# nz0001na/MorphGANformer

Measured on AMD Instinct MI355X. Metric: latent-projection iters/sec @1024^2, k=17 latents, higher is better.
Workload: dtype f32; 1 GPU; configs[1]: single 1024x1024 face per GPU, Wing+LPIPS(squeeze)+MSE literal-mode projection step, noise_mode=random, seeded synthetic weights/targets/landmarks; k=17, z_dim=32, targets_per_gpu=1, parallelism=pair-sharded x1, graph_replay=True, loss_generator_overlap=True, steps_per_forward=32

## Files before the change

### include/mgf.h

```cpp
#ifndef MGF_H_
#define MGF_H_

#include <stdint.h>

#ifdef __cplusplus
extern "C" {
#endif

typedef void* mgf_stream_t;

enum { MGF_OK = 0, MGF_EINVAL = -1, MGF_EUNSUPPORTED = -2, MGF_ELAUNCH = -3, MGF_ETOOBIG = -4 };
enum { MGF_F32 = 0, MGF_F64 = 1, MGF_F16 = 2 };
enum { MGF_FILTER_SEPARABLE = 2 };
enum { MGF_FILTER_LARGE = 4 };
enum { MGF_ACT_LINEAR = 1, MGF_ACT_RELU = 2, MGF_ACT_LRELU = 3, MGF_ACT_TANH = 4, MGF_ACT_SIGMOID = 5,
       MGF_ACT_ELU = 6, MGF_ACT_SELU = 7, MGF_ACT_SOFTPLUS = 8, MGF_ACT_SWISH = 9,
       MGF_ACT_RELU_POST = 10 };

const char* mgf_last_error(void);
int mgf_version(void);
int mgf_device_ok(void);

int mgf_bias_act(void* y, const void* x, const void* b, const void* xref, const void* yref, const void* dy,
                 int dtype, int64_t numel, int64_t step_b, int64_t size_b,
// ... 80 lines not shown

int mgf_conv3x3s2_few_inputs_f32(float* y, const float* x, const float* w, const float* bias, int32_t n, int32_t cin, int32_t in_h,
                                 int32_t in_w, int32_t cout, int32_t relu, mgf_stream_t stream);
int mgf_tconv3x3s2_few_outputs_f32(float* y, const float* x, const float* wp, int32_t n, int32_t cin, int32_t h, int32_t w, int32_t cout,
                                   int32_t cout_pad, int32_t pitch, int64_t y_plane, int64_t y_batch, mgf_stream_t stream);
int mgf_conv3x3_winograd3_up2res_f32(float* y, const float* x, const float* u, const float* in_scale, const float* out_scale,
                                     const float* residual_low, int32_t n, int32_t cin, int32_t h, int32_t w, int32_t cout,
                                     int32_t out_scale_stride, const mgf_epilogue* ep, mgf_stream_t stream);
int mgf_winograd3_force_shape(int32_t shape);
int mgf_conv3x3_winograd3_rgb_f32(float* rgb_out, const float* x, const float* u, const float* in_scale, const float* out_scale,
                                  const float* rgb_w, const float* rgb_bias, int32_t n, int32_t cin, int32_t h, int32_t w, int32_t cout,
                                  int32_t out_scale_stride, int32_t rgb_channels, mgf_stream_t stream);
int mgf_conv3x3_winograd_f32(float* y, const float* x, const float* u, const float* in_scale, const float* out_scale, int32_t n,
                             int32_t cin, int32_t h, int32_t w, int32_t cout, int32_t out_scale_stride, const mgf_epilogue* ep,
                             mgf_stream_t stream);

int mgf_tconv3x3s2_border_f32(float* t, const float* x, const float* wp, const float* in_scale, const float* out_scale, int32_t n,
                              int32_t cin, int32_t h, int32_t w, int32_t cout, int32_t cout_pad, int64_t t_pitch, int64_t t_plane,
                              int64_t t_batch, int64_t out_scale_stride, mgf_stream_t stream);

int mgf_tconv3x3s2_winograd_f32(float* t, const float* x, const float* u, const float* in_scale, const float* out_scale, int32_t n,
                                int32_t cin, int32_t h, int32_t w, int32_t cout, int32_t pitch, int64_t t_plane, int64_t t_batch,
                                int64_t out_scale_stride, mgf_stream_t stream);
int mgf_tconv_winograd_weights_f32(float* u, const float* w, int32_t cout, int32_t cin, double gain, mgf_stream_t stream);

int mgf_pack_conv_weights(float* wp, float* wsq, const float* w, int32_t cout, int32_t cin, int32_t kh, int32_t kw,
                          int32_t cout_pad, float gain, int32_t flip, mgf_stream_t stream);

typedef struct mgf_style_job {
    const float* aff_w;
    const float* aff_b;
    const float* wsq;
    float* s;
    float* d;
    int32_t cin, cout;
    int32_t w_offset;
    float aff_gain, style_gain;
} mgf_style_job;
int mgf_demod_f32(float* d, const float* s, const float* wsq, int32_t n, int32_t cin, int32_t cout, mgf_stream_t stream);
int mgf_demod_bwd_f32(float* ds, const float* dd, const float* d, const float* s, const float* wsq, int32_t n, int32_t cin, int32_t cout,
                      mgf_stream_t stream);
int mgf_style_demod(const mgf_style_job* job, const float* ws, int64_t ws_stride_n, int32_t n, int32_t wdim, mgf_stream_t stream);
int mgf_style_demod_multi(const mgf_style_job* jobs_dev, int32_t njobs, const float* ws, int64_t ws_stride_n,
                          int32_t n, int32_t wdim, int32_t max_cin, mgf_stream_t stream);

int mgf_duplex_attention(float* y, const float* x, const float* wqc, const float* spos, const float* vwb,
// ... 199 lines not shown
```

### morphganformer_amd/_lib.py

```python
from __future__ import annotations

import ctypes as C
import os

import torch

HERE = os.path.dirname(os.path.abspath(__file__))
LIB_PATH = os.environ.get("MGF_LIB_PATH") or os.path.join(HERE, "libmgf_hip.so")

MGF_F32, MGF_F64, MGF_F16 = 0, 1, 2
ACT_IDS = {"linear": 1, "relu": 2, "lrelu": 3, "tanh": 4, "sigmoid": 5, "elu": 6, "selu": 7, "softplus": 8, "swish": 9,
           "relu_post": 10}
MAX_TAPS = 9

i32, i64, f32, f64, vp = C.c_int32, C.c_int64, C.c_float, C.c_double, C.c_void_p


class Epilogue(C.Structure):
    _fields_ = [("bias", vp), ("noise", vp), ("noise_strength", vp), ("noise_n", i32), ("act", i32), ("alpha", f32),
                ("gain", f32), ("residual", vp)]


class ConvDesc(C.Structure):
    _fields_ = [("n", i32), ("cin", i32), ("in_h", i32), ("in_w", i32), ("cout", i32), ("cout_pad", i32),
# ... 36 lines not shown
    "mgf_version": (C.c_int, []),
    "mgf_device_ok": (C.c_int, []),
    "mgf_bias_act": (C.c_int, [vp, vp, vp, vp, vp, vp, C.c_int, i64, i64, i64, C.c_int, C.c_int, f32, f32, f32, vp]),
    "mgf_upfirdn2d": (C.c_int, [vp, vp, vp, C.c_int, i32, i32, i32, i32, i64, i64, i64, i64, i32, i32, i64, i64, i64, i64,
                                i32, i32, i32, i32, i32, i32, i32, i32, i32, i32, i32, f32, C.POINTER(Epilogue), vp]),
    "mgf_conv_taps_f32": (C.c_int, [vp, vp, vp, vp, vp, C.POINTER(ConvDesc), C.POINTER(Epilogue), vp]),
    "mgf_conv_taps_bf16x3_f32": (C.c_int, [vp, vp, vp, vp, vp, C.POINTER(ConvDesc), C.POINTER(Epilogue), vp]),
    "mgf_tconv3x3s2_border_f32": (C.c_int, [vp, vp, vp, vp, vp, i32, i32, i32, i32, i32, i32, i64, i64, i64, i64, vp]),
    "mgf_tconv3x3s2_winograd_f32": (C.c_int, [vp, vp, vp, vp, vp, i32, i32, i32, i32, i32, i32, i64, i64, i64, vp]),
    "mgf_tconv_winograd_weights_f32": (C.c_int, [vp, vp, i32, i32, C.c_double, vp]),
    "mgf_winograd_weights_f32": (C.c_int, [vp, vp, i32, i32, f32, vp]),
    "mgf_conv3x3_winograd_f32": (C.c_int, [vp, vp, vp, vp, vp, i32, i32, i32, i32, i32, i32, C.POINTER(Epilogue), vp]),
    "mgf_winograd2_weights_f32": (C.c_int, [vp, vp, i32, i32, f32, vp]),
    "mgf_conv3x3_winograd2_f32": (C.c_int, [vp, vp, vp, vp, vp, i32, i32, i32, i32, i32, i32, C.POINTER(Epilogue), vp]),
    "mgf_conv3x3_winograd2_rgb_f32": (C.c_int, [vp, vp, vp, vp, vp, vp, vp, i32, i32, i32, i32, i32, i32, i32, vp]),
    "mgf_conv3x3_winograd3_f32": (C.c_int, [vp, vp, vp, vp, vp, i32, i32, i32, i32, i32, i32, C.POINTER(Epilogue), vp]),
    "mgf_conv1x1_f32": (C.c_int, [vp, vp, vp, vp, i32, i32, i32, i32, i32, i64, i32, C.POINTER(Epilogue), vp]),
    "mgf_conv3x3s2_few_inputs_f32": (C.c_int, [vp, vp, vp, vp, i32, i32, i32, i32, i32, i32, vp]),
    "mgf_tconv3x3s2_few_outputs_f32": (C.c_int, [vp, vp, vp, i32, i32, i32, i32, i32, i32, i32, i64, i64, vp]),
    "mgf_conv1x1_force_shape": (C.c_int, [i32]),
    "mgf_conv3x3_winograd3_slice_f32": (C.c_int, [vp, vp, vp, vp, vp, i32, i32, i32, i32, i32, i32, i64, i32, C.POINTER(Epilogue), vp]),
    "mgf_conv3x3_winograd3_up2res_f32": (C.c_int, [vp, vp, vp, vp, vp, vp, i32, i32, i32, i32, i32, i32, C.POINTER(Epilogue), vp]),
    "mgf_winograd3_force_shape": (C.c_int, [i32]),
    "mgf_conv3x3_winograd3_rgb_f32": (C.c_int, [vp, vp, vp, vp, vp, vp, vp, i32, i32, i32, i32, i32, i32, i32, vp]),
    "mgf_conv3x3_winograd2_slice_f32": (C.c_int, [vp, vp, vp, vp, vp, i32, i32, i32, i32, i32, i32, i64, i32, C.POINTER(Epilogue), vp]),
    "mgf_pack_conv_weights": (C.c_int, [vp, vp, vp, i32, i32, i32, i32, i32, f32, i32, vp]),
    "mgf_conv_profile_begin": (C.c_int, []),
    "mgf_conv_profile_end": (C.c_int, [C.POINTER(ConvProfRec), i32]),
    "mgf_demod_f32": (C.c_int, [vp, vp, vp, i32, i32, i32, vp]),
    "mgf_demod_bwd_f32": (C.c_int, [vp, vp, vp, vp, vp, i32, i32, i32, vp]),
    "mgf_style_demod": (C.c_int, [C.POINTER(StyleJob), vp, i64, i32, i32, vp]),
    "mgf_style_demod_multi": (C.c_int, [vp, i32, vp, i64, i32, i32, i32, vp]),
    "mgf_duplex_attention": (C.c_int, [vp, vp, vp, vp, vp, i32, i32, i32, i32, C.POINTER(Epilogue), i32, vp, vp, vp]),
    "mgf_att_map_upsample_f32": (C.c_int, [vp, vp, i32, i32, i32, i32, i32, i32, vp]),
    "mgf_attn_values": (C.c_int, [C.POINTER(AttnJob), vp, i64, i64, i32, i32, i32, vp]),
    "mgf_attn_values_multi": (C.c_int, [vp, i32, vp, i64, i64, i32, i32, i32, vp]),
    "mgf_randn_f32": (C.c_int, [vp, i64, C.c_uint64, vp, vp]),
    "mgf_rgb_weights_f32": (C.c_int, [vp, vp, vp, i32, i32, i32, vp]),
    "mgf_torgb_compose_weights_f32": (C.c_int, [vp, vp, vp, vp, vp, vp, i32, i32, i32, i32, vp]),
    "mgf_conv3x3_few_outputs_f32": (C.c_int, [vp, vp, vp, vp, i32, i32, i32, i32, i32, vp]),
    "mgf_mapping_param_floats": (i64, [i32, i32, i32]),
    "mgf_mapping_forward": (C.c_int, [vp, vp, vp, i32, i32, i32, i32, i32, vp]),
    "mgf_reduce_scratch_floats": (i64, []),
    "mgf_mse_f32": (C.c_int, [vp, vp, vp, i32, i64, i64, f32, i32, vp, vp]),
    "mgf_dssim_scratch_bytes": (i64, [i32, i32, i32, i32]),
    "mgf_dssim_u8_f32": (C.c_int, [vp, vp, vp, i32, i32, i32, i32, i64, f32, f32, i32, vp, vp]),
# ... 131 lines not shown
```

### morphganformer_amd/conv.py

```python
from __future__ import annotations

import ctypes as C
import os
from dataclasses import dataclass

import torch

from . import _lib


def round_up(v: int, m: int) -> int:
    return (v + m - 1) // m * m


def profile_begin():
    _lib.check(_lib.lib().mgf_conv_profile_begin(), "conv_profile_begin")


def profile_end(max_recs=4096):
    recs = (_lib.ConvProfRec * max_recs)()
    n = _lib.lib().mgf_conv_profile_end(recs, max_recs)
    if n < 0:
        _lib.check(n, "conv_profile_end")
    return [(recs[i].kernel.decode(), recs[i].flops, recs[i].seconds, recs[i].ksplit, recs[i].bytes) for i in range(min(n, max_recs))]
# ... 370 lines not shown
                                                      _lib.stream_ptr()), "conv3x3_few_outputs")
    return out


TCONV_WINO = os.environ.get("MGF_TCONV_WINO", "1") != "0"
TCONV_WINO_MIN_WGS = 4096


def tconv_winograd_weights(w: torch.Tensor, gain: float = 1.0) -> torch.Tensor:
    _lib.require_gpu(w)
    w = w.contiguous().float()
    cout, cin, kh, kw = w.shape
    assert (kh, kw) == (3, 3) and cin % 4 == 0
    u = torch.empty([25, cin // 4, cout, 4], dtype=torch.float32, device=w.device)
    _lib.check(_lib.lib().mgf_tconv_winograd_weights_f32(u.data_ptr(), w.data_ptr(), cout, cin, float(gain), _lib.stream_ptr()),
               "tconv_winograd_weights")
    return u


def tconv_winograd_ok(n, cin, h, w, cout, out, bf=None) -> bool:
    return bool(TCONV_WINO and SPLIT_TCONV_BORDER and bf is None and h % 2 == 0 and w % 2 == 0 and min(h, w) >= TCONV_SPLIT_MIN and cin % 4 == 0 and cout % 32 == 0
                and out.shape[3] % 4 == 0 and out.data_ptr() % 16 == 0
                and n * -(-h // 4) * -(-w // 32) * (cout // 32) >= TCONV_WINO_MIN_WGS)


def tconv3x3s2_forward(x, pc: PackedConv, in_scale=None, out_scale=None, out=None, bf=None, wt=None):
    _lib.require_gpu(x, pc.wp, in_scale, out_scale, out, wt)
    assert pc.kh == 3 and pc.kw == 3 and x.dtype == torch.float32 and x.is_contiguous()
    n, cin, h, w = x.shape
    oh, ow = 2 * h + 1, 2 * w + 1
    if out is None:
        out = torch.empty([n, pc.cout, oh, tconv_pitch(w)], dtype=torch.float32, device=x.device)
    pitch = out.shape[3]
    assert out.is_contiguous() and tuple(out.shape) == (n, pc.cout, oh, pitch) and pitch >= ow and pitch % 4 == 0
    if NARROW_CONV and pc.cout <= 4 and in_scale is None and out_scale is None:
        rc = _lib.lib().mgf_tconv3x3s2_few_outputs_f32(out.data_ptr(), x.data_ptr(), pc.wp.data_ptr(), n, cin, h, w, pc.cout, pc.cout_pad,
                                                       pitch, oh * pitch, pc.cout * oh * pitch, _lib.stream_ptr())
        _lib.check(rc, "tconv3x3s2_few_outputs")
        return out[:, :, :, :ow]
    if wt is not None and tconv_winograd_ok(n, cin, h, w, pc.cout, out, bf):
        assert tuple(wt.shape) == (25, cin // 4, pc.cout, 4)
        os_stride = 0 if out_scale is None else out_scale.stride(0) if out_scale.ndim == 2 else 0
        rc = _lib.lib().mgf_tconv3x3s2_winograd_f32(out.data_ptr(), x.data_ptr(), wt.data_ptr(), _lib.ptr(in_scale), _lib.ptr(out_scale), n, cin, h,
                                                    w, pc.cout, pitch, oh * pitch, pc.cout * oh * pitch, os_stride, _lib.stream_ptr())
        _lib.check(rc, "tconv3x3s2_winograd")
        rc = _lib.lib().mgf_tconv3x3s2_border_f32(out.data_ptr(), x.data_ptr(), pc.wp.data_ptr(), _lib.ptr(in_scale), _lib.ptr(out_scale),
# ... 41 lines not shown
```

### morphganformer_amd/csrc/wino_tconv.hip

```cpp
#include "mgf_common.h"
#include <algorithm>
#include <type_traits>

namespace {

typedef float f32x16 __attribute__((ext_vector_type(16)));
typedef float v2f __attribute__((ext_vector_type(2)));

constexpr int WTCK = 4;
constexpr int WTFW = 34;
constexpr int WTFH = 5;
constexpr int WTFP = WTFH * WTFW;
constexpr int WTNP = 25;
constexpr int WTXS = 14;
__constant__ float wt_ones[WTCK] = {1.f, 1.f, 1.f, 1.f};

struct WinoTParams {
    float* t;
    const float* x;
    const float* u;
    const float* in_scale;
    const float* out_scale;
    int n, cin, h, w, cout, os_stride, pitch;
    int tiles_x, tiles_y, co_tiles;
    int xcd_per;
    int64_t t_plane, t_batch;
};

__global__ __launch_bounds__(256, 2) void wino_tconv_kernel(WinoTParams p) {
    constexpr int CST = 256, RAW = WTCK * CST;
    extern __shared__ float lds[];
    float* const raw0 = lds;
    float* const raw1 = raw0 + RAW;
    const int tid = threadIdx.x, lane = tid & 63;
    const int a = __builtin_amdgcn_readfirstlane(tid >> 6);
    const int l31 = lane & 31, half = lane >> 5;
    const int tx = l31 & 15, ty = l31 >> 4;

    int b_ = blockIdx.x;
    if (p.xcd_per > 0) {
        b_ = (b_ & 7) * p.xcd_per + (b_ >> 3);
        if (b_ >= p.n * p.tiles_x * p.tiles_y * p.co_tiles) return;
    }
    const int cot = b_ % p.co_tiles; b_ /= p.co_tiles;
    const int ptx = b_ % p.tiles_x; b_ /= p.tiles_x;
    const int pty = b_ % p.tiles_y;
    const int n = b_ / p.tiles_y;
    const int co0 = cot * 32, iy0 = pty * 4, ix0 = ptx * 32;
    const int plane = p.h * p.w;
    const float* xn = p.x + (int64_t)n * p.cin * plane;
    const float* sc = p.in_scale ? p.in_scale + (int64_t)n * p.cin : nullptr;
    const int nck = p.cin / WTCK;

    const __amdgpu_buffer_rsrc_t rx = __builtin_amdgcn_make_buffer_rsrc((void*)xn, 0, p.cin * plane * 4, 0x00020000);
    const __amdgpu_buffer_rsrc_t ru = __builtin_amdgcn_make_buffer_rsrc((void*)p.u, 0, WTNP * p.cin * p.cout * 4, 0x00020000);
    const __amdgpu_buffer_rsrc_t rnull = __builtin_amdgcn_make_buffer_rsrc((void*)p.u, 0, 0, 0x00020000);
    unsigned xoff;
    {
        const int r = tid / WTFW, q = tid - r * WTFW;
        const int iy = iy0 - 1 + r, ix = ix0 - 1 + q;
        xoff = (tid < WTFP && iy >= 0 && iy < p.h && ix >= 0 && ix < p.w) ? (unsigned)(iy * p.w + ix) * 4u : 0xFFFFFFF0u;
    }
    const unsigned aoff = (unsigned)(((co0 + l31) * WTCK + half * 2) * 4);
    const int upos = nck * p.cout * WTCK * 4;
    const int ubase_row = 5 * a * upos, ubase_col = (20 + a) * upos, ubase_sh = 24 * upos + (a & 1) * 4;

    float xr[WTCK];
    auto load_x = [&](float (&dst)[WTCK], int c0, bool live = true) {
        const __amdgpu_buffer_rsrc_t r = live ? rx : rnull;
#pragma unroll
        for (int j = 0; j < WTCK; ++j) dst[j] = __builtin_bit_cast(float, __builtin_amdgcn_raw_buffer_load_b32(r, xoff, (c0 + j) * plane * 4, 0));
    };
    typedef const float __attribute__((address_space(4)))* cfp4;
    const cfp4 sbase = sc ? (cfp4)sc : (cfp4)wt_ones;
    const int sstep = sc ? 1 : 0;
    auto load_s = [&](float (&dst)[WTCK], int c0) {
#pragma unroll
        for (int j = 0; j < WTCK; ++j) dst[j] = sbase[c0 * sstep + j];
    };
    auto park_x = [&](float* R, const float (&src)[WTCK], const float (&sv)[WTCK]) {
#pragma unroll
        for (int j = 0; j < WTCK; ++j) R[j * CST + tid] = src[j] * sv[j];
    };
    struct Aop { v2f q[6]; float s; };
    auto load_a = [&](Aop& dst, int c0, bool live = true) {
        const int soff = c0 * p.cout * 4;
        const __amdgpu_buffer_rsrc_t r = live ? ru : rnull;
#pragma unroll
        for (int b = 0; b < 5; ++b)
            dst.q[b] = __builtin_bit_cast(v2f, __builtin_amdgcn_raw_buffer_load_b64(r, aoff, ubase_row + b * upos + soff, 0));
        dst.q[5] = __builtin_bit_cast(v2f, __builtin_amdgcn_raw_buffer_load_b64(r, aoff, ubase_col + soff, 0));
        dst.s = __builtin_bit_cast(float, __builtin_amdgcn_raw_buffer_load_b32(r, aoff, ubase_sh + soff, 0));
    };
    const int pr = a == 0 ? 0 : (a == 2 ? 2 : 1);
    const float sg = (a == 0 || a == 2) ? -1.f : 0.f;
    const int px = a == 0 ? 0 : (a == 2 ? 2 : 1);
    const float sgf = (a == 0 || a == 2) ? -1.f : 0.f;
    auto transform = [&](float (&B)[2][6], const float* R) {
#pragma unroll
        for (int kk = 0; kk < 2; ++kk) {
            const float* src = R + (half + 2 * kk) * CST + 2 * ty * WTFW + 2 * tx;
            const float* rp = src + pr * WTFW;
            const float* r1 = src + WTFW;
            const float* r2 = src + 2 * WTFW;
            const v2f p01 = *reinterpret_cast<const v2f*>(rp), q01 = *reinterpret_cast<const v2f*>(r1), f01 = *reinterpret_cast<const v2f*>(r2);
            const float p2 = rp[2], q2 = r1[2], f2 = r2[2];
            const v2f sg2 = {sg, sg};
            const v2f e01 = p01 + sg2 * q01;
            const float e2 = p2 + sg * q2;
            B[kk][0] = e01.x - e01.y;
            B[kk][1] = e01.y;
            B[kk][2] = e2 - e01.y;
            B[kk][3] = e2;
            const float fp = px == 0 ? f01.x : (px == 2 ? f2 : f01.y);
            B[kk][4] = fp + sgf * f01.y;
            B[kk][5] = f2;
        }
    };

    f32x16 acc[6];
    f32x16 accs = {};
    constexpr int BI[5] = {0, 1, 2, 1, 3};
    auto mfma_chunk = [&](const Aop& A, const float (&B)[2][6], auto first_tag, auto parity_tag) {
        constexpr bool FIRST = decltype(first_tag)::value;
        constexpr int PAR = decltype(parity_tag)::value;
#pragma unroll
        for (int b = 0; b < 6; ++b) {
            const int bi = b < 5 ? BI[b] : 4;
            acc[b] = __builtin_amdgcn_mfma_f32_32x32x2f32(A.q[b].x, B[0][bi], FIRST ? f32x16{} : acc[b], 0, 0, 0);
            acc[b] = __builtin_amdgcn_mfma_f32_32x32x2f32(A.q[b].y, B[1][bi], acc[b], 0, 0, 0);
        }
        if ((a >> 1) == PAR) {
            const float bs = (a & 1) ? B[1][5] : B[0][5];
            accs = __builtin_amdgcn_mfma_f32_32x32x2f32(A.s, bs, accs, 0, 0, 0);
        }
    };

    const int nchunks = nck;
    const int last = nchunks - 1;
    auto chunk0 = [&](int i) { return (i < last ? i : last) * WTCK; };
    Aop A0, A1;
    float B0[2][6], B1[2][6];
    float sv[WTCK];
    {
        float xa[WTCK], xb[WTCK], sa_[WTCK], sb_[WTCK];
        load_s(sv, chunk0(2));
        load_x(xa, 0);
        load_a(A0, 0);
        load_x(xb, chunk0(1));
        load_x(xr, chunk0(2));
        load_s(sa_, 0);
        load_s(sb_, chunk0(1));
        park_x(raw0, xa, sa_);
        park_x(raw1, xb, sb_);
        __syncthreads();
        transform(B0, raw0);
        __syncthreads();
    }
    auto body = [&](int i, Aop& Acur, Aop& Anxt, float (&Bcur)[2][6], float (&Bnxt)[2][6], float* raw_nxt, float* raw_park, auto first_tag,
                    auto parity_tag) {
        load_a(Anxt, chunk0(i + 1), i + 1 < nchunks);
        __builtin_amdgcn_sched_barrier(0);
        transform(Bnxt, raw_nxt);
        mfma_chunk(Acur, Bcur, first_tag, parity_tag);
        __builtin_amdgcn_sched_barrier(0);
        park_x(raw_park, xr, sv);
        load_x(xr, chunk0(i + 3), i + 3 < nchunks);
        load_s(sv, chunk0(i + 3));
        __syncthreads();
    };
    using P0 = std::integral_constant<int, 0>;
    using P1 = std::integral_constant<int, 1>;
    body(0, A0, A1, B0, B1, raw1, raw0, std::true_type{}, P0{});
    if (1 < nchunks) body(1, A1, A0, B1, B0, raw0, raw1, std::false_type{}, P1{});
    for (int it = 2; it < nchunks; it += 2) {
        body(it, A0, A1, B0, B1, raw1, raw0, std::false_type{}, P0{});
        if (it + 1 < nchunks) body(it + 1, A1, A0, B1, B0, raw0, raw1, std::false_type{}, P1{});
    }

    float R[4][16];
#pragma unroll
    for (int v = 0; v < 16; ++v) {
        R[0][v] = acc[0][v] + acc[1][v];
        R[1][v] = acc[3][v];
        R[2][v] = acc[1][v] + acc[2][v];
        R[3][v] = acc[4][v];
    }
    float* const xch = lds;
    auto put = [&](int slot, const float* vals) {
        float* dst = xch + slot * 1024 + lane;
#pragma unroll
        for (int v = 0; v < 16; ++v) dst[v * 64] = vals[v];
    };
    float colv[16], shv[16];
#pragma unroll
    for (int v = 0; v < 16; ++v) { colv[v] = acc[5][v]; shv[v] = accs[v]; }
    if (a == 1) {
#pragma unroll
        for (int j = 0; j < 4; ++j) put(j, R[j]);
        put(10, colv);
        put(11, shv);
    } else if (a == 2) {
#pragma unroll
        for (int j = 0; j < 4; ++j) put(4 + j, R[j]);
    } else if (a == 0) {
        put(8, colv);
        put(9, shv);
    } else {
        put(12, colv);
        put(13, shv);
    }
    __syncthreads();
    const float* xl = xch + lane;
    float Y[4][16];
    if (a == 0 || a == 1) {
        const int s0 = a == 0 ? 0 : 4;
#pragma unroll
        for (int j = 0; j < 4; ++j)
#pragma unroll
            for (int v = 0; v < 16; ++v) Y[j][v] = R[j][v] + xl[(s0 + j) * 1024 + v * 64];
    } else if (a == 2) {
#pragma unroll
        for (int v = 0; v < 16; ++v) {
            const float m51 = xl[8 * 1024 + v * 64], m52 = xl[10 * 1024 + v * 64], m54 = xl[12 * 1024 + v * 64];
            Y[0][v] = m51 + m52;
            Y[1][v] = m54;
            Y[2][v] = m52 + colv[v];
            Y[3][v] = (xl[9 * 1024 + v * 64] + xl[11 * 1024 + v * 64]) + (shv[v] + xl[13 * 1024 + v * 64]);
        }
    } else {
#pragma unroll
        for (int j = 0; j < 4; ++j)
#pragma unroll
            for (int v = 0; v < 16; ++v) Y[j][v] = R[j][v];
    }
    const int orow = a == 0 ? 0 : (a == 1 ? 2 : (a == 2 ? 3 : 1));
    const int by = iy0 + 2 * ty, bx = ix0 + 2 * tx;
    const bool ok = by < p.h && bx < p.w;
    const int cob = co0 + 4 * half;
    const float* osc = p.out_scale ? p.out_scale + (int64_t)n * p.os_stride + cob : nullptr;
    const unsigned toff = ok ? (unsigned)(((int64_t)cob * p.t_plane + (int64_t)(2 * by + orow) * p.pitch + 2 * bx) * 4) : 0xFFFFFFF0u;
    typedef unsigned v4u __attribute__((ext_vector_type(4)));
    const __amdgpu_buffer_rsrc_t rt = __builtin_amdgcn_make_buffer_rsrc((void*)(p.t + (int64_t)n * p.t_batch), 0,
                                                                       (int)((int64_t)p.cout * p.t_plane * 4), 0x00020000);
#pragma unroll
    for (int v = 0; v < 16; ++v) {
        const int cl = (v & 3) + 8 * (v >> 2);
        const float s = osc ? osc[cl] : 1.f;
        const v4u o = {__builtin_bit_cast(unsigned, Y[0][v] * s), __builtin_bit_cast(unsigned, Y[1][v] * s),
                       __builtin_bit_cast(unsigned, Y[2][v] * s), __builtin_bit_cast(unsigned, Y[3][v] * s)};
        __builtin_amdgcn_raw_buffer_store_b128(o, rt, toff, (int)(cl * p.t_plane * 4), 0);
    }
}

__global__ __launch_bounds__(256) void wino_tconv_weights_kernel(float* u, const float* w, int cout, int cin, double gain) {
    const int64_t total = (int64_t)cout * cin;
    for (int64_t i = (int64_t)blockIdx.x * 256 + threadIdx.x; i < total; i += (int64_t)gridDim.x * 256) {
        const int co = (int)(i % cout), ci = (int)(i / cout);
        const float* g = w + ((int64_t)co * cin + ci) * 9;
        double t[5][3];
#pragma unroll
        for (int v = 0; v < 3; ++v) {
            const double g0 = g[v], g1 = g[3 + v], g2 = g[6 + v];
            t[0][v] = g2;
            t[1][v] = g0 + g2;
            t[2][v] = g0;
            t[3][v] = g1;
            t[4][v] = g1;
        }
        const int cl = ci & 3, slot = 2 * (cl & 1) + (cl >> 1);
        const int64_t pl = (int64_t)cin * cout;
        float* dst = u + (((int64_t)(ci >> 2)) * cout + co) * 4 + slot;
#pragma unroll
        for (int r = 0; r < 5; ++r) {
            const double o[5] = {t[r][2], t[r][0] + t[r][2], t[r][0], t[r][1], t[r][1]};
#pragma unroll
            for (int c = 0; c < 5; ++c) dst[(5 * r + c) * pl] = (float)(o[c] * gain);
        }
    }
}

}

extern "C" int mgf_tconv_winograd_weights_f32(float* u, const float* w, int32_t cout, int32_t cin, double gain, mgf_stream_t stream) {
    MGF_REQUIRE(u && w && cout >= 1 && cin >= 1, MGF_EINVAL, "tconv_winograd_weights: bad arguments");
    MGF_REQUIRE(cin % WTCK == 0, MGF_EUNSUPPORTED, "tconv_winograd_weights: cin must be a multiple of %d (got %d)", WTCK, cin);
    hipLaunchKernelGGL(wino_tconv_weights_kernel, dim3(mgf_stream_grid((int64_t)cout * cin, 256, 1)), dim3(256), 0, (hipStream_t)stream, u, w, cout,
                       cin, gain);
    MGF_CHECK_LAUNCH("tconv_winograd_weights");
    return MGF_OK;
}

extern "C" int mgf_tconv3x3s2_winograd_f32(float* t, const float* x, const float* u, const float* in_scale, const float* out_scale, int32_t n,
                                           int32_t cin, int32_t h, int32_t w, int32_t cout, int32_t pitch, int64_t t_plane, int64_t t_batch,
                                           int64_t out_scale_stride, mgf_stream_t stream) {
    MGF_REQUIRE(t && x && u && n >= 1 && cin >= 1 && cout >= 1 && h >= 2 && w >= 2, MGF_EINVAL, "tconv3x3s2_winograd: bad arguments");
    MGF_REQUIRE(cin % WTCK == 0 && cout % 32 == 0, MGF_EUNSUPPORTED, "tconv3x3s2_winograd: cin must be a multiple of %d and cout of 32 (got %d, %d)",
                WTCK, cin, cout);
    MGF_REQUIRE(h % 2 == 0 && w % 2 == 0, MGF_EUNSUPPORTED, "tconv3x3s2_winograd: even map sides only (got %dx%d)", h, w);
    MGF_REQUIRE(pitch >= 2 * w + 1 && pitch % 4 == 0 && t_plane >= (int64_t)(2 * h + 1) * pitch && t_plane % 4 == 0 && t_batch % 4 == 0 &&
                    t_batch >= (int64_t)cout * t_plane, MGF_EINVAL, "tconv3x3s2_winograd: bad workspace layout");
    MGF_REQUIRE(((uintptr_t)t % 16) == 0 && ((uintptr_t)u % 16) == 0, MGF_EINVAL, "tconv3x3s2_winograd: t and u must be 16-byte aligned");
    MGF_REQUIRE((int64_t)cin * h * w <= INT32_MAX / 4 && (int64_t)WTNP * cin * cout <= INT32_MAX / 4 && (int64_t)cout * t_plane <= INT32_MAX / 4,
                MGF_ETOOBIG, "tconv3x3s2_winograd: one sample / the weight planes must stay below 2 GiB (32-bit buffer offsets)");
    WinoTParams p{};
    p.t = t; p.x = x; p.u = u; p.in_scale = in_scale; p.out_scale = out_scale;
    p.n = n; p.cin = cin; p.h = h; p.w = w; p.cout = cout; p.os_stride = (int)out_scale_stride; p.pitch = pitch;
    p.t_plane = t_plane; p.t_batch = t_batch;
    p.tiles_x = (int)mgf_cdiv(w, 32);
    p.tiles_y = (int)mgf_cdiv(h, 4);
    p.co_tiles = cout / 32;
    int64_t blocks = (int64_t)n * p.tiles_x * p.tiles_y * p.co_tiles;
    MGF_REQUIRE(blocks <= INT32_MAX - 8, MGF_ETOOBIG, "tconv3x3s2_winograd: too many workgroups");
    p.xcd_per = 0;
    if ((int64_t)WTNP * cin * cout * 4 <= (4 << 20) && blocks >= 16) {
        p.xcd_per = (int)((blocks + 7) / 8);
        blocks = (int64_t)p.xcd_per * 8;
    }
    const size_t lds = std::max<size_t>((size_t)2 * WTCK * 256, (size_t)WTXS * 16 * 64) * sizeof(float);
    static bool attr_set = false;
    if (!attr_set) {
        hipError_t e = hipFuncSetAttribute((const void*)wino_tconv_kernel, hipFuncAttributeMaxDynamicSharedMemorySize, 65536);
        if (e != hipSuccess) { mgf_set_error("tconv3x3s2_winograd: cannot raise dynamic LDS: %s", hipGetErrorString(e)); return MGF_ELAUNCH; }
        attr_set = true;
    }
    mgf_prof_external_begin((hipStream_t)stream, "wino_tconv_kernel", 2.0 * 9 * cin * (double)cout * h * w * n,
                            4.0 * ((double)n * cin * h * w + 9.0 * cin * cout + (double)n * cout * 4.0 * h * w));
    hipLaunchKernelGGL(wino_tconv_kernel, dim3((unsigned)blocks), dim3(256), lds, (hipStream_t)stream, p);
    mgf_prof_external_end((hipStream_t)stream);
    MGF_CHECK_LAUNCH("tconv3x3s2_winograd");
    return MGF_OK;
}
```

Baseline: 767.9 iters/s.

## Add persistent and deeper-prefetch variants of the Winograd transposed-conv kernel

Templates the Winograd stride-2 transposed-conv kernel on prefetch depth (one or two chunks ahead) and on a persistent mode. In persistent mode each workgroup loops over several output tiles and prefetches the next tile's operands across the tile boundary, with a separate LDS region for the epilogue exchange. A runtime selector (force call or env knob) picks the form. The default stays the one-shot, one-ahead form, so the new schedules are opt-in. They trade more registers and LDS for hiding per-tile startup and load latency.

```diff
diff --git a/include/mgf.h b/include/mgf.h
--- a/include/mgf.h
+++ b/include/mgf.h
@@ -126,6 +126,12 @@
 int mgf_tconv3x3s2_winograd_f32(float* t, const float* x, const float* u, const float* in_scale, const float* out_scale, int32_t n,
                                 int32_t cin, int32_t h, int32_t w, int32_t cout, int32_t pitch, int64_t t_plane, int64_t t_batch,
                                 int64_t out_scale_stride, mgf_stream_t stream);
+#define MGF_TCONV_WINO_ONESHOT1 1
+#define MGF_TCONV_WINO_ONESHOT2 2
+#define MGF_TCONV_WINO_PERSISTENT 3
+#define MGF_TCONV_WINO_PERSISTENT1 4
+int mgf_tconv_winograd_force_form(int32_t form);
+int mgf_tconv_winograd_form(int32_t n, int32_t cin, int32_t h, int32_t w, int32_t cout);
 int mgf_tconv_winograd_weights_f32(float* u, const float* w, int32_t cout, int32_t cin, double gain, mgf_stream_t stream);
 
 int mgf_pack_conv_weights(float* wp, float* wsq, const float* w, int32_t cout, int32_t cin, int32_t kh, int32_t kw,
diff --git a/morphganformer_amd/_lib.py b/morphganformer_amd/_lib.py
--- a/morphganformer_amd/_lib.py
+++ b/morphganformer_amd/_lib.py
@@ -82,6 +82,8 @@
     "mgf_conv3x3_winograd3_slice_f32": (C.c_int, [vp, vp, vp, vp, vp, i32, i32, i32, i32, i32, i32, i64, i32, C.POINTER(Epilogue), vp]),
     "mgf_conv3x3_winograd3_up2res_f32": (C.c_int, [vp, vp, vp, vp, vp, vp, i32, i32, i32, i32, i32, i32, C.POINTER(Epilogue), vp]),
     "mgf_winograd3_force_shape": (C.c_int, [i32]),
+    "mgf_tconv_winograd_force_form": (C.c_int, [i32]),
+    "mgf_tconv_winograd_form": (C.c_int, [i32, i32, i32, i32, i32]),
     "mgf_conv3x3_winograd3_rgb_f32": (C.c_int, [vp, vp, vp, vp, vp, vp, vp, i32, i32, i32, i32, i32, i32, i32, vp]),
     "mgf_conv3x3_winograd2_slice_f32": (C.c_int, [vp, vp, vp, vp, vp, i32, i32, i32, i32, i32, i32, i64, i32, C.POINTER(Epilogue), vp]),
     "mgf_pack_conv_weights": (C.c_int, [vp, vp, vp, i32, i32, i32, i32, i32, f32, i32, vp]),
diff --git a/morphganformer_amd/conv.py b/morphganformer_amd/conv.py
--- a/morphganformer_amd/conv.py
+++ b/morphganformer_amd/conv.py
@@ -416,6 +416,14 @@
     return bool(TCONV_WINO and SPLIT_TCONV_BORDER and bf is None and h % 2 == 0 and w % 2 == 0 and min(h, w) >= TCONV_SPLIT_MIN and cin % 4 == 0 and cout % 32 == 0
                 and out.shape[3] % 4 == 0 and out.data_ptr() % 16 == 0
                 and n * -(-h // 4) * -(-w // 32) * (cout // 32) >= TCONV_WINO_MIN_WGS)
+
+
+def tconv_winograd_force_form(form: int) -> None:
+    _lib.check(_lib.lib().mgf_tconv_winograd_force_form(int(form)), "tconv_winograd_force_form")
+
+
+def tconv_winograd_form(n, cin, h, w, cout) -> int:
+    return int(_lib.lib().mgf_tconv_winograd_form(n, cin, h, w, cout))
 
 
 def tconv3x3s2_forward(x, pc: PackedConv, in_scale=None, out_scale=None, out=None, bf=None, wt=None):
diff --git a/morphganformer_amd/csrc/wino_tconv.hip b/morphganformer_amd/csrc/wino_tconv.hip
--- a/morphganformer_amd/csrc/wino_tconv.hip
+++ b/morphganformer_amd/csrc/wino_tconv.hip
@@ -23,75 +23,112 @@
     const float* out_scale;
     int n, cin, h, w, cout, os_stride, pitch;
     int tiles_x, tiles_y, co_tiles;
+    int items;
     int xcd_per;
     int64_t t_plane, t_batch;
 };
 
+template <int DEPTH, bool PERSIST>
 __global__ __launch_bounds__(256, 2) void wino_tconv_kernel(WinoTParams p) {
+    static_assert(DEPTH == 1 || DEPTH == 2, "operand rings one or two chunks ahead");
     constexpr int CST = 256, RAW = WTCK * CST;
     extern __shared__ float lds[];
     float* const raw0 = lds;
     float* const raw1 = raw0 + RAW;
+    float* const xch = PERSIST ? raw1 + RAW : lds;
     const int tid = threadIdx.x, lane = tid & 63;
     const int a = __builtin_amdgcn_readfirstlane(tid >> 6);
     const int l31 = lane & 31, half = lane >> 5;
     const int tx = l31 & 15, ty = l31 >> 4;
-
-    int b_ = blockIdx.x;
-    if (p.xcd_per > 0) {
-        b_ = (b_ & 7) * p.xcd_per + (b_ >> 3);
-        if (b_ >= p.n * p.tiles_x * p.tiles_y * p.co_tiles) return;
-    }
-    const int cot = b_ % p.co_tiles; b_ /= p.co_tiles;
-    const int ptx = b_ % p.tiles_x; b_ /= p.tiles_x;
-    const int pty = b_ % p.tiles_y;
-    const int n = b_ / p.tiles_y;
-    const int co0 = cot * 32, iy0 = pty * 4, ix0 = ptx * 32;
     const int plane = p.h * p.w;
-    const float* xn = p.x + (int64_t)n * p.cin * plane;
-    const float* sc = p.in_scale ? p.in_scale + (int64_t)n * p.cin : nullptr;
     const int nck = p.cin / WTCK;
-
-    const __amdgpu_buffer_rsrc_t rx = __builtin_amdgcn_make_buffer_rsrc((void*)xn, 0, p.cin * plane * 4, 0x00020000);
+    const int last = nck - 1;
+
+    auto item_index = [&](int k) -> int {
+        if constexpr (!PERSIST) {
+            int b = blockIdx.x;
+            if (p.xcd_per > 0) b = (b & 7) * p.xcd_per + (b >> 3);
+            return (k == 0 && b < p.items) ? b : -1;
+        } else {
+            if (p.xcd_per > 0) {
+                const int s = (int)(blockIdx.x >> 3) + k * (int)(gridDim.x >> 3);
+                const int b = (int)(blockIdx.x & 7) * p.xcd_per + s;
+                return (s < p.xcd_per && b < p.items) ? b : -1;
+            }
+            const int b = (int)blockIdx.x + k * (int)gridDim.x;
+            return b < p.items ? b : -1;
+        }
+    };
+    struct Item { int n, co0, iy0, ix0, live; };
+    auto decode = [&](int b) -> Item {
+        Item it{0, 0, 0, 0, 0};
+        if (b < 0) return it;
+        const int cot = b % p.co_tiles; b /= p.co_tiles;
+        const int ptx = b % p.tiles_x; b /= p.tiles_x;
+        const int pty = b % p.tiles_y;
+        it.n = b / p.tiles_y; it.co0 = cot * 32; it.iy0 = pty * 4; it.ix0 = ptx * 32; it.live = 1;
+        return it;
+    };
+    Item icur = decode(item_index(0));
+    if (!icur.live) return;
+    Item inxt = PERSIST ? decode(item_index(1)) : Item{0, 0, 0, 0, 0};
+
+    typedef const float __attribute__((address_space(4)))* cfp4;
     const __amdgpu_buffer_rsrc_t ru = __builtin_amdgcn_make_buffer_rsrc((void*)p.u, 0, WTNP * p.cin * p.cout * 4, 0x00020000);
     const __amdgpu_buffer_rsrc_t rnull = __builtin_amdgcn_make_buffer_rsrc((void*)p.u, 0, 0, 0x00020000);
-    unsigned xoff;
-    {
-        const int r = tid / WTFW, q = tid - r * WTFW;
-        const int iy = iy0 - 1 + r, ix = ix0 - 1 + q;
-        xoff = (tid < WTFP && iy >= 0 && iy < p.h && ix >= 0 && ix < p.w) ? (unsigned)(iy * p.w + ix) * 4u : 0xFFFFFFF0u;
-    }
-    const unsigned aoff = (unsigned)(((co0 + l31) * WTCK + half * 2) * 4);
+    const int fr = tid / WTFW, fq = tid - fr * WTFW;
+    struct Src { __amdgpu_buffer_rsrc_t rx, ra; unsigned xoff; int abase; cfp4 s; };
+    auto make_src = [&](const Item& it) -> Src {
+        Src s;
+        s.rx = it.live ? __builtin_amdgcn_make_buffer_rsrc((void*)(p.x + (int64_t)it.n * p.cin * plane), 0, p.cin * plane * 4, 0x00020000) : rnull;
+        s.ra = it.live ? ru : rnull;
+        const int iy = it.iy0 - 1 + fr, ix = it.ix0 - 1 + fq;
+        s.xoff = (tid < WTFP && iy >= 0 && iy < p.h && ix >= 0 && ix < p.w) ? (unsigned)(iy * p.w + ix) * 4u : 0xFFFFFFF0u;
+        s.abase = it.co0 * WTCK * 4;
+        s.s = p.in_scale ? (cfp4)(p.in_scale + (int64_t)it.n * p.cin) : (cfp4)wt_ones;
+        return s;
+    };
+    Src scur = make_src(icur), snxt = make_src(inxt);
+    int c = 0;
+    const int sstep = p.in_scale ? 1 : 0;
+
+    const unsigned aoff = (unsigned)((l31 * WTCK + half * 2) * 4);
     const int upos = nck * p.cout * WTCK * 4;
     const int ubase_row = 5 * a * upos, ubase_col = (20 + a) * upos, ubase_sh = 24 * upos + (a & 1) * 4;
 
-    float xr[WTCK];
-    auto load_x = [&](float (&dst)[WTCK], int c0, bool live = true) {
-        const __amdgpu_buffer_rsrc_t r = live ? rx : rnull;
-#pragma unroll
-        for (int j = 0; j < WTCK; ++j) dst[j] = __builtin_bit_cast(float, __builtin_amdgcn_raw_buffer_load_b32(r, xoff, (c0 + j) * plane * 4, 0));
-    };
-    typedef const float __attribute__((address_space(4)))* cfp4;
-    const cfp4 sbase = sc ? (cfp4)sc : (cfp4)wt_ones;
-    const int sstep = sc ? 1 : 0;
-    auto load_s = [&](float (&dst)[WTCK], int c0) {
-#pragma unroll
-        for (int j = 0; j < WTCK; ++j) dst[j] = sbase[c0 * sstep + j];
+#define WT_POS(d)                                                                                                                     \
+    const int q_ = c + (d);                                                                                                           \
+    const bool cu_ = q_ < nck;                                                                                                        \
+    const int ch_ = cu_ ? q_ : min(q_ - nck, last);
+    auto load_x = [&](float (&dst)[WTCK], int d) {
+        WT_POS(d)
+        const __amdgpu_buffer_rsrc_t r = cu_ ? scur.rx : snxt.rx;
+        const unsigned vo = cu_ ? scur.xoff : snxt.xoff;
+#pragma unroll
+        for (int j = 0; j < WTCK; ++j) dst[j] = __builtin_bit_cast(float, __builtin_amdgcn_raw_buffer_load_b32(r, vo, (ch_ * WTCK + j) * plane * 4, 0));
+    };
+    auto load_s = [&](float (&dst)[WTCK], int d) {
+        WT_POS(d)
+        const cfp4 sb = cu_ ? scur.s : snxt.s;
+#pragma unroll
+        for (int j = 0; j < WTCK; ++j) dst[j] = sb[ch_ * WTCK * sstep + j];
     };
     auto park_x = [&](float* R, const float (&src)[WTCK], const float (&sv)[WTCK]) {
 #pragma unroll
         for (int j = 0; j < WTCK; ++j) R[j * CST + tid] = src[j] * sv[j];
     };
     struct Aop { v2f q[6]; float s; };
-    auto load_a = [&](Aop& dst, int c0, bool live = true) {
-        const int soff = c0 * p.cout * 4;
-        const __amdgpu_buffer_rsrc_t r = live ? ru : rnull;
+    auto load_a = [&](Aop& dst, int d) {
+        WT_POS(d)
+        const __amdgpu_buffer_rsrc_t r = cu_ ? scur.ra : snxt.ra;
+        const int soff = ch_ * p.cout * WTCK * 4 + (cu_ ? scur.abase : snxt.abase);
 #pragma unroll
         for (int b = 0; b < 5; ++b)
             dst.q[b] = __builtin_bit_cast(v2f, __builtin_amdgcn_raw_buffer_load_b64(r, aoff, ubase_row + b * upos + soff, 0));
         dst.q[5] = __builtin_bit_cast(v2f, __builtin_amdgcn_raw_buffer_load_b64(r, aoff, ubase_col + soff, 0));
         dst.s = __builtin_bit_cast(float, __builtin_amdgcn_raw_buffer_load_b32(r, aoff, ubase_sh + soff, 0));
     };
+#undef WT_POS
     const int pr = a == 0 ? 0 : (a == 2 ? 2 : 1);
     const float sg = (a == 0 || a == 2) ? -1.f : 0.f;
     const int px = a == 0 ? 0 : (a == 2 ? 2 : 1);
@@ -119,15 +156,20 @@
     };
 
     f32x16 acc[6];
-    f32x16 accs = {};
+    f32x16 accs;
+    auto zero_acc = [&]() {
+#pragma unroll
+        for (int b = 0; b < 6; ++b) acc[b] = f32x16{};
+        accs = f32x16{};
+    };
+    zero_acc();
     constexpr int BI[5] = {0, 1, 2, 1, 3};
-    auto mfma_chunk = [&](const Aop& A, const float (&B)[2][6], auto first_tag, auto parity_tag) {
-        constexpr bool FIRST = decltype(first_tag)::value;
+    auto mfma_chunk = [&](const Aop& A, const float (&B)[2][6], auto parity_tag) {
         constexpr int PAR = decltype(parity_tag)::value;
 #pragma unroll
         for (int b = 0; b < 6; ++b) {
             const int bi = b < 5 ? BI[b] : 4;
-            acc[b] = __builtin_amdgcn_mfma_f32_32x32x2f32(A.q[b].x, B[0][bi], FIRST ? f32x16{} : acc[b], 0, 0, 0);
+            acc[b] = __builtin_amdgcn_mfma_f32_32x32x2f32(A.q[b].x, B[0][bi], acc[b], 0, 0, 0);
             acc[b] = __builtin_amdgcn_mfma_f32_32x32x2f32(A.q[b].y, B[1][bi], acc[b], 0, 0, 0);
         }
         if ((a >> 1) == PAR) {
@@ -136,121 +178,159 @@
         }
     };
 
-    const int nchunks = nck;
-    const int last = nchunks - 1;
-    auto chunk0 = [&](int i) { return (i < last ? i : last) * WTCK; };
-    Aop A0, A1;
+    auto epilogue = [&](const Item& it) {
+        float R[4][16];
+#pragma unroll
+        for (int v = 0; v < 16; ++v) {
+            R[0][v] = acc[0][v] + acc[1][v];
+            R[1][v] = acc[3][v];
+            R[2][v] = acc[1][v] + acc[2][v];
+            R[3][v] = acc[4][v];
+        }
+        auto put = [&](int slot, const float* vals) {
+            float* dst = xch + slot * 1024 + lane;
+#pragma unroll
+            for (int v = 0; v < 16; ++v) dst[v * 64] = vals[v];
+        };
+        float colv[16], shv[16];
+#pragma unroll
+        for (int v = 0; v < 16; ++v) { colv[v] = acc[5][v]; shv[v] = accs[v]; }
+        if (a == 1) {
+#pragma unroll
+            for (int j = 0; j < 4; ++j) put(j, R[j]);
+            put(10, colv);
+            put(11, shv);
+        } else if (a == 2) {
+#pragma unroll
+            for (int j = 0; j < 4; ++j) put(4 + j, R[j]);
+        } else if (a == 0) {
+            put(8, colv);
+            put(9, shv);
+        } else {
+            put(12, colv);
+            put(13, shv);
+        }
+        __syncthreads();
+        const float* xl = xch + lane;
+        float (&Y)[4][16] = R;
+        if (a == 0 || a == 1) {
+            const int s0 = a == 0 ? 0 : 4;
+#pragma unroll
+            for (int j = 0; j < 4; ++j)
+#pragma unroll
+                for (int v = 0; v < 16; ++v) Y[j][v] = R[j][v] + xl[(s0 + j) * 1024 + v * 64];
+        } else if (a == 2) {
+#pragma unroll
+            for (int v = 0; v < 16; ++v) {
+                const float m51 = xl[8 * 1024 + v * 64], m52 = xl[10 * 1024 + v * 64], m54 = xl[12 * 1024 + v * 64];
+                Y[0][v] = m51 + m52;
+                Y[1][v] = m54;
+                Y[2][v] = m52 + colv[v];
+                Y[3][v] = (xl[9 * 1024 + v * 64] + xl[11 * 1024 + v * 64]) + (shv[v] + xl[13 * 1024 + v * 64]);
+            }
+        }
+        const int orow = a == 0 ? 0 : (a == 1 ? 2 : (a == 2 ? 3 : 1));
+        const int by = it.iy0 + 2 * ty, bx = it.ix0 + 2 * tx;
+        const bool ok = by < p.h && bx < p.w;
+        const int cob = it.co0 + 4 * half;
+        const float* osc = p.out_scale ? p.out_scale + (int64_t)it.n * p.os_stride + cob : nullptr;
+        const unsigned toff = ok ? (unsigned)(((int64_t)cob * p.t_plane + (int64_t)(2 * by + orow) * p.pitch + 2 * bx) * 4) : 0xFFFFFFF0u;
+        typedef unsigned v4u __attribute__((ext_vector_type(4)));
+        const __amdgpu_buffer_rsrc_t rt = __builtin_amdgcn_make_buffer_rsrc((void*)(p.t + (int64_t)it.n * p.t_batch), 0,
+                                                                           (int)((int64_t)p.cout * p.t_plane * 4), 0x00020000);
+#pragma unroll
+        for (int v = 0; v < 16; ++v) {
+            const int cl = (v & 3) + 8 * (v >> 2);
+            const float s = osc ? osc[cl] : 1.f;
+            const v4u o = {__builtin_bit_cast(unsigned, Y[0][v] * s), __builtin_bit_cast(unsigned, Y[1][v] * s),
+                           __builtin_bit_cast(unsigned, Y[2][v] * s), __builtin_bit_cast(unsigned, Y[3][v] * s)};
+            __builtin_amdgcn_raw_buffer_store_b128(o, rt, toff, (int)(cl * p.t_plane * 4), 0);
+        }
+    };
+
+    Aop A0, A1, A2;
     float B0[2][6], B1[2][6];
-    float sv[WTCK];
+    float xr[WTCK], sv[WTCK], xr1[WTCK], sv1[WTCK];
     {
         float xa[WTCK], xb[WTCK], sa_[WTCK], sb_[WTCK];
-        load_s(sv, chunk0(2));
+        load_s(sv, 2);
         load_x(xa, 0);
         load_a(A0, 0);
-        load_x(xb, chunk0(1));
-        load_x(xr, chunk0(2));
+        load_x(xb, 1);
+        if constexpr (DEPTH == 2) load_a(A1, 1);
+        load_x(xr, 2);
+        if constexpr (DEPTH == 2) {
+            load_x(xr1, 3);
+            load_s(sv1, 3);
+        }
         load_s(sa_, 0);
-        load_s(sb_, chunk0(1));
+        load_s(sb_, 1);
         park_x(raw0, xa, sa_);
         park_x(raw1, xb, sb_);
         __syncthreads();
         transform(B0, raw0);
         __syncthreads();
     }
-    auto body = [&](int i, Aop& Acur, Aop& Anxt, float (&Bcur)[2][6], float (&Bnxt)[2][6], float* raw_nxt, float* raw_park, auto first_tag,
-                    auto parity_tag) {
-        load_a(Anxt, chunk0(i + 1), i + 1 < nchunks);
+    auto advance = [&](int& k) {
+        if constexpr (PERSIST) {
+            if (c == last) {
+                epilogue(icur);
+                zero_acc();
+                ++k;
+                icur = inxt;
+                scur = snxt;
+                inxt = decode(item_index(k + 1));
+                snxt = make_src(inxt);
+                c = 0;
+                return;
+            }
+        }
+        ++c;
+    };
+    auto body = [&](Aop& Acur, Aop& Afar, float (&Bcur)[2][6], float (&Bnxt)[2][6], float* raw_nxt, float* raw_park, float (&xq)[WTCK],
+                    float (&sq)[WTCK], auto parity_tag) {
+        load_a(Afar, DEPTH);
         __builtin_amdgcn_sched_barrier(0);
         transform(Bnxt, raw_nxt);
-        mfma_chunk(Acur, Bcur, first_tag, parity_tag);
+        mfma_chunk(Acur, Bcur, parity_tag);
         __builtin_amdgcn_sched_barrier(0);
-        park_x(raw_park, xr, sv);
-        load_x(xr, chunk0(i + 3), i + 3 < nchunks);
-        load_s(sv, chunk0(i + 3));
+        park_x(raw_park, xq, sq);
+        load_x(xq, DEPTH + 2);
+        load_s(sq, DEPTH + 2);
         __syncthreads();
     };
     using P0 = std::integral_constant<int, 0>;
     using P1 = std::integral_constant<int, 1>;
-    body(0, A0, A1, B0, B1, raw1, raw0, std::true_type{}, P0{});
-    if (1 < nchunks) body(1, A1, A0, B1, B0, raw0, raw1, std::false_type{}, P1{});
-    for (int it = 2; it < nchunks; it += 2) {
-        body(it, A0, A1, B0, B1, raw1, raw0, std::false_type{}, P0{});
-        if (it + 1 < nchunks) body(it + 1, A1, A0, B1, B0, raw0, raw1, std::false_type{}, P1{});
-    }
-
-    float R[4][16];
-#pragma unroll
-    for (int v = 0; v < 16; ++v) {
-        R[0][v] = acc[0][v] + acc[1][v];
-        R[1][v] = acc[3][v];
-        R[2][v] = acc[1][v] + acc[2][v];
-        R[3][v] = acc[4][v];
-    }
-    float* const xch = lds;
-    auto put = [&](int slot, const float* vals) {
-        float* dst = xch + slot * 1024 + lane;
-#pragma unroll
-        for (int v = 0; v < 16; ++v) dst[v * 64] = vals[v];
-    };
-    float colv[16], shv[16];
-#pragma unroll
-    for (int v = 0; v < 16; ++v) { colv[v] = acc[5][v]; shv[v] = accs[v]; }
-    if (a == 1) {
-#pragma unroll
-        for (int j = 0; j < 4; ++j) put(j, R[j]);
-        put(10, colv);
-        put(11, shv);
-    } else if (a == 2) {
-#pragma unroll
-        for (int j = 0; j < 4; ++j) put(4 + j, R[j]);
-    } else if (a == 0) {
-        put(8, colv);
-        put(9, shv);
+    int k = 0;
+    int nitems = 1;
+    if constexpr (PERSIST) {
+        if (p.xcd_per > 0) {
+            const int s0 = (int)(blockIdx.x >> 3), ns = (int)(gridDim.x >> 3);
+            const int lim = min(p.xcd_per, p.items - (int)(blockIdx.x & 7) * p.xcd_per);
+            nitems = (lim - s0 + ns - 1) / ns;
+        } else {
+            nitems = (p.items - (int)blockIdx.x + (int)gridDim.x - 1) / (int)gridDim.x;
+        }
+    }
+    const int S = nitems * nck;
+    if constexpr (DEPTH == 2) {
+        for (int g = 0; g < S; g += 6) {
+            body(A0, A2, B0, B1, raw1, raw0, xr, sv, P0{});
+            advance(k);
+            if (g + 1 < S) { body(A1, A0, B1, B0, raw0, raw1, xr1, sv1, P1{}); advance(k); }
+            if (g + 2 < S) { body(A2, A1, B0, B1, raw1, raw0, xr, sv, P0{}); advance(k); }
+            if (g + 3 < S) { body(A0, A2, B1, B0, raw0, raw1, xr1, sv1, P1{}); advance(k); }
+            if (g + 4 < S) { body(A1, A0, B0, B1, raw1, raw0, xr, sv, P0{}); advance(k); }
+            if (g + 5 < S) { body(A2, A1, B1, B0, raw0, raw1, xr1, sv1, P1{}); advance(k); }
+        }
     } else {
-        put(12, colv);
-        put(13, shv);
-    }
-    __syncthreads();
-    const float* xl = xch + lane;
-    float Y[4][16];
-    if (a == 0 || a == 1) {
-        const int s0 = a == 0 ? 0 : 4;
-#pragma unroll
-        for (int j = 0; j < 4; ++j)
-#pragma unroll
-            for (int v = 0; v < 16; ++v) Y[j][v] = R[j][v] + xl[(s0 + j) * 1024 + v * 64];
-    } else if (a == 2) {
-#pragma unroll
-        for (int v = 0; v < 16; ++v) {
-            const float m51 = xl[8 * 1024 + v * 64], m52 = xl[10 * 1024 + v * 64], m54 = xl[12 * 1024 + v * 64];
-            Y[0][v] = m51 + m52;
-            Y[1][v] = m54;
-            Y[2][v] = m52 + colv[v];
-            Y[3][v] = (xl[9 * 1024 + v * 64] + xl[11 * 1024 + v * 64]) + (shv[v] + xl[13 * 1024 + v * 64]);
-        }
-    } else {
-#pragma unroll
-        for (int j = 0; j < 4; ++j)
-#pragma unroll
-            for (int v = 0; v < 16; ++v) Y[j][v] = R[j][v];
-    }
-    const int orow = a == 0 ? 0 : (a == 1 ? 2 : (a == 2 ? 3 : 1));
-    const int by = iy0 + 2 * ty, bx = ix0 + 2 * tx;
-    const bool ok = by < p.h && bx < p.w;
-    const int cob = co0 + 4 * half;
-    const float* osc = p.out_scale ? p.out_scale + (int64_t)n * p.os_stride + cob : nullptr;
-    const unsigned toff = ok ? (unsigned)(((int64_t)cob * p.t_plane + (int64_t)(2 * by + orow) * p.pitch + 2 * bx) * 4) : 0xFFFFFFF0u;
-    typedef unsigned v4u __attribute__((ext_vector_type(4)));
-    const __amdgpu_buffer_rsrc_t rt = __builtin_amdgcn_make_buffer_rsrc((void*)(p.t + (int64_t)n * p.t_batch), 0,
-                                                                       (int)((int64_t)p.cout * p.t_plane * 4), 0x00020000);
-#pragma unroll
-    for (int v = 0; v < 16; ++v) {
-        const int cl = (v & 3) + 8 * (v >> 2);
-        const float s = osc ? osc[cl] : 1.f;
-        const v4u o = {__builtin_bit_cast(unsigned, Y[0][v] * s), __builtin_bit_cast(unsigned, Y[1][v] * s),
-                       __builtin_bit_cast(unsigned, Y[2][v] * s), __builtin_bit_cast(unsigned, Y[3][v] * s)};
-        __builtin_amdgcn_raw_buffer_store_b128(o, rt, toff, (int)(cl * p.t_plane * 4), 0);
-    }
+        for (int g = 0; g < S; g += 2) {
+            body(A0, A1, B0, B1, raw1, raw0, xr, sv, P0{});
+            advance(k);
+            if (g + 1 < S) { body(A1, A0, B1, B0, raw0, raw1, xr, sv, P1{}); advance(k); }
+        }
+    }
+    if constexpr (!PERSIST) epilogue(icur);
 }
 
 __global__ __launch_bounds__(256) void wino_tconv_weights_kernel(float* u, const float* w, int cout, int cin, double gain) {
@@ -280,6 +360,30 @@
     }
 }
 
+}
+
+static int g_tconv_forced_form = 0;
+
+extern "C" int mgf_tconv_winograd_force_form(int32_t form) {
+    MGF_REQUIRE(form >= 0 && form <= 4, MGF_EINVAL,
+                "tconv_winograd_force_form: 0 (auto), 1 / 2 = one-shot with operands one / two chunks ahead, 3 / 4 = persistent with operands two / "
+                "one chunks ahead wherever the shape admits it (got %d)", form);
+    g_tconv_forced_form = form;
+    return MGF_OK;
+}
+
+static int tconv_winograd_form(int32_t n, int32_t cin, int32_t h, int32_t w, int32_t cout) {
+    const int64_t items = (int64_t)n * mgf_cdiv(h, 4) * mgf_cdiv(w, 32) * (cout / 32);
+    const bool persist_ok = cin / WTCK >= 4 && items >= 512;
+    static const int env_form = [] { const char* e = mgf_knob("MGF_TCONV_WINO_FORM"); return e ? atoi(e) : 0; }();
+    const int f = g_tconv_forced_form ? g_tconv_forced_form : env_form;
+    if (f == MGF_TCONV_WINO_PERSISTENT || f == MGF_TCONV_WINO_PERSISTENT1) return persist_ok ? f : MGF_TCONV_WINO_ONESHOT2;
+    if (f == MGF_TCONV_WINO_ONESHOT1 || f == MGF_TCONV_WINO_ONESHOT2) return f;
+    return MGF_TCONV_WINO_ONESHOT1;
+}
+
+extern "C" int mgf_tconv_winograd_form(int32_t n, int32_t cin, int32_t h, int32_t w, int32_t cout) {
+    return tconv_winograd_form(n, cin, h, w, cout);
 }
 
 extern "C" int mgf_tconv_winograd_weights_f32(float* u, const float* w, int32_t cout, int32_t cin, double gain, mgf_stream_t stream) {
@@ -312,21 +416,50 @@
     p.co_tiles = cout / 32;
     int64_t blocks = (int64_t)n * p.tiles_x * p.tiles_y * p.co_tiles;
     MGF_REQUIRE(blocks <= INT32_MAX - 8, MGF_ETOOBIG, "tconv3x3s2_winograd: too many workgroups");
+    p.items = (int)blocks;
+    const int form = tconv_winograd_form(n, cin, h, w, cout);
+    const bool xcd = (int64_t)WTNP * cin * cout * 4 <= (4 << 20) && blocks >= 16;
     p.xcd_per = 0;
-    if ((int64_t)WTNP * cin * cout * 4 <= (4 << 20) && blocks >= 16) {
+    const bool persist = form == MGF_TCONV_WINO_PERSISTENT || form == MGF_TCONV_WINO_PERSISTENT1;
+    if (persist) {
+        static const int slots = [] {
+            int dev = 0, cus = 0;
+            if (hipGetDevice(&dev) != hipSuccess || hipDeviceGetAttribute(&cus, hipDeviceAttributeMultiprocessorCount, dev) != hipSuccess) cus = 256;
+            return 2 * std::max(cus, 4);
+        }();
+        int64_t g = std::min<int64_t>(slots, blocks);
+        if (xcd) {
+            g = std::max<int64_t>(8, g / 8 * 8);
+            p.xcd_per = (int)((blocks + 7) / 8);
+        }
+        blocks = g;
+    } else if (xcd) {
         p.xcd_per = (int)((blocks + 7) / 8);
         blocks = (int64_t)p.xcd_per * 8;
     }
-    const size_t lds = std::max<size_t>((size_t)2 * WTCK * 256, (size_t)WTXS * 16 * 64) * sizeof(float);
+    const size_t lds = (persist ? (size_t)2 * WTCK * 256 + (size_t)WTXS * 16 * 64
+                                :std::max<size_t>((size_t)2 * WTCK * 256, (size_t)WTXS * 16 * 64)) * sizeof(float);
     static bool attr_set = false;
     if (!attr_set) {
-        hipError_t e = hipFuncSetAttribute((const void*)wino_tconv_kernel, hipFuncAttributeMaxDynamicSharedMemorySize, 65536);
+        hipError_t e = hipFuncSetAttribute((const void*)wino_tconv_kernel<1, false>, hipFuncAttributeMaxDynamicSharedMemorySize, 65536);
+        if (e == hipSuccess) e = hipFuncSetAttribute((const void*)wino_tconv_kernel<2, false>, hipFuncAttributeMaxDynamicSharedMemorySize, 65536);
+        if (e == hipSuccess) e = hipFuncSetAttribute((const void*)wino_tconv_kernel<2, true>, hipFuncAttributeMaxDynamicSharedMemorySize, 65536);
+        if (e == hipSuccess) e = hipFuncSetAttribute((const void*)wino_tconv_kernel<1, true>, hipFuncAttributeMaxDynamicSharedMemorySize, 65536);
         if (e != hipSuccess) { mgf_set_error("tconv3x3s2_winograd: cannot raise dynamic LDS: %s", hipGetErrorString(e)); return MGF_ELAUNCH; }
         attr_set = true;
     }
-    mgf_prof_external_begin((hipStream_t)stream, "wino_tconv_kernel", 2.0 * 9 * cin * (double)cout * h * w * n,
+    static const char* const names[5] = {"", "wino_tconv_kernel<1, false>", "wino_tconv_kernel<2, false>", "wino_tconv_kernel<2, true>",
+                                         "wino_tconv_kernel<1, true>"};
+    mgf_prof_external_begin((hipStream_t)stream, names[form], 2.0 * 9 * cin * (double)cout * h * w * n,
                             4.0 * ((double)n * cin * h * w + 9.0 * cin * cout + (double)n * cout * 4.0 * h * w));
-    hipLaunchKernelGGL(wino_tconv_kernel, dim3((unsigned)blocks), dim3(256), lds, (hipStream_t)stream, p);
+    const dim3 grid((unsigned)blocks), blk(256);
+    hipStream_t st = (hipStream_t)stream;
+    switch (form) {
+        case MGF_TCONV_WINO_ONESHOT1: hipLaunchKernelGGL((wino_tconv_kernel<1, false>), grid, blk, lds, st, p); break;
+        case MGF_TCONV_WINO_ONESHOT2: hipLaunchKernelGGL((wino_tconv_kernel<2, false>), grid, blk, lds, st, p); break;
+        case MGF_TCONV_WINO_PERSISTENT: hipLaunchKernelGGL((wino_tconv_kernel<2, true>), grid, blk, lds, st, p); break;
+        default: hipLaunchKernelGGL((wino_tconv_kernel<1, true>), grid, blk, lds, st, p); break;
+    }
     mgf_prof_external_end((hipStream_t)stream);
     MGF_CHECK_LAUNCH("tconv3x3s2_winograd");
     return MGF_OK;
```

New measurement: 763.0 iters/s (median of 2 runs). No clear change (-0.6%).
